# BarisYazici/deep-rl-grasping

Hardware: NVIDIA H100
Metric: SAC grad-steps/sec (batch 256, 64x64 depth) (higher is better)
Workload: dtype bf16x3 (fp32-faithful split, f32 accumulate)

## Files before the change

deep-rl-grasping_b200/csrc/engine_v2.cu:

```cuda
#include <cuda_bf16.h>

#include <algorithm>
#include <cstdio>
#include <cstdlib>
#include <cstring>

#include "sac_internal.cuh"

namespace b2g {
namespace {

struct Gather2Args {
  GatherArgs g;
  uint16_t* a1[2][3];
  uint16_t* fp[3][3];
  int KF, Ci, OH, OW;
};

__device__ __forceinline__ void split3(float y, uint16_t& p0, uint16_t& p1, uint16_t& p2) {
  const __nv_bfloat16 h0 = __float2bfloat16_rn(y);
  const float r1 = y - __bfloat162float(h0);
  const __nv_bfloat16 h1 = __float2bfloat16_rn(r1);
  const float r2 = r1 - __bfloat162float(h1);
  p0 = __bfloat16_as_ushort(h0); p1 = __bfloat16_as_ushort(h1); p2 = __bfloat16_as_ushort(__float2bfloat16_rn(r2));
}

__global__ void __launch_bounds__(512) gather2_kernel(Gather2Args a) {
  extern __shared__ uint16_t sm_planes[];
  const GatherArgs& g = a.g;
  const int b = blockIdx.x, which = blockIdx.y, tid = threadIdx.x;
  const int Ci = a.Ci, HW = g.H * g.W, npx = HW * Ci;
  const int Ec = npx + 4;
  long long slot = b;
  if (g.indices) slot = g.indices[b];
  else if (g.rng_counters) {
    slot = philox_slot(g.seed, (unsigned long long)g.rng_counters[4], b, (unsigned long long)g.rng_counters[5]);
    if (g.indices_out && which == 0 && tid == 0) g.indices_out[b] = (int)slot;
  }
  const float* __restrict__ src = (which ? g.next_obs : g.obs) + (size_t)slot * Ec;
  const double clip_obs = g.normc[1];
  const bool norm_obs = g.normc[3] != 0.0;
  const float scale = g.scale;
  const int rowe = g.W * Ci, pitch = rowe + 8, plane_e = g.H * pitch;
  for (int e4 = tid; e4 < (npx >> 2); e4 += blockDim.x) {
    const float4 v = *reinterpret_cast<const float4*>(src + 4 * e4);
    float y[4] = {v.x, v.y, v.z, v.w};
    if (norm_obs) {
      const double2 m0 = *reinterpret_cast<const double2*>(g.mean + 4 * e4), m1 = *reinterpret_cast<const double2*>(g.mean + 4 * e4 + 2);
      const double2 i0 = *reinterpret_cast<const double2*>(g.var + 4 * e4), i1 = *reinterpret_cast<const double2*>(g.var + 4 * e4 + 2);
      y[0] = (float)fmin(fmax(((double)y[0] - m0.x) * i0.x, -clip_obs), clip_obs);
      y[1] = (float)fmin(fmax(((double)y[1] - m0.y) * i0.y, -clip_obs), clip_obs);
      y[2] = (float)fmin(fmax(((double)y[2] - m1.x) * i1.x, -clip_obs), clip_obs);
      y[3] = (float)fmin(fmax(((double)y[3] - m1.y) * i1.y, -clip_obs), clip_obs);
    }
    uint16_t p[3][4];
#pragma unroll
    for (int j = 0; j < 4; ++j) split3(y[j] / scale, p[0][j], p[1][j], p[2][j]);
#pragma unroll
    for (int pl = 0; pl < 3; ++pl) {
      const uint2 w = make_uint2((uint32_t)p[pl][0] | ((uint32_t)p[pl][1] << 16), (uint32_t)p[pl][2] | ((uint32_t)p[pl][3] << 16));
      const int e = 4 * e4, row = e / rowe, col = e - row * rowe;
      *reinterpret_cast<uint2*>(sm_planes + pl * plane_e + row * pitch + col) = w;
    }
  }
  if (tid == 0) {
    float yy = src[npx];
    if (norm_obs) yy = (float)fmin(fmax(((double)yy - g.mean[npx]) * g.var[npx], -clip_obs), clip_obs);
    yy = yy / scale;
    uint16_t p0, p1, p2;
    split3(yy, p0, p1, p2);
    const size_t fo = (size_t)b * g.FS + g.feat_col, po = (size_t)b * a.KF + g.feat_col;
    if (which) { g.F_t[fo] = yy; a.fp[2][0][po] = p0; a.fp[2][1][po] = p1; a.fp[2][2][po] = p2; }
    else {
      g.F_pi[fo] = yy; g.F_v[fo] = yy;
      a.fp[0][0][po] = p0; a.fp[0][1][po] = p1; a.fp[0][2][po] = p2;
      a.fp[1][0][po] = p0; a.fp[1][1][po] = p1; a.fp[1][2][po] = p2;
    }
  }
  __syncthreads();
  const int seg = 8 * Ci;
  const int K1 = 64 * Ci, nruns = a.OH * a.OW * 8;
  const size_t img = (size_t)b * a.OH * a.OW * K1;
  for (int i = tid; i < nruns * (seg / 8); i += blockDim.x) {
    const int part = i % (seg / 8), run = i / (seg / 8);
    const int ky = run & 7, patch = run >> 3;
    const int oy = patch / a.OW, ox = patch - oy * a.OW;
    const int so = (4 * oy + ky) * pitch + 4 * ox * Ci + 8 * part;
    const size_t go = img + (size_t)patch * K1 + ky * seg + 8 * part;
#pragma unroll
    for (int pl = 0; pl < 3; ++pl) {
      const uint16_t* sp = sm_planes + pl * plane_e + so;
      const uint2 lo = *reinterpret_cast<const uint2*>(sp), hi = *reinterpret_cast<const uint2*>(sp + 4);
      *reinterpret_cast<uint4*>(a.a1[which][pl] + go) = make_uint4(lo.x, lo.y, hi.x, hi.y);
    }
  }
  if (which == 0 && g.act) {
    const int feat_dim = g.feat_col + 1;
    if (tid < g.n_act) {
      const float av = g.act[slot * g.n_act + tid];
      g.F_v[(size_t)b * g.FS + feat_dim + tid] = av;
      uint16_t p0, p1, p2;
      split3(av, p0, p1, p2);
      const size_t po = (size_t)b * a.KF + feat_dim + tid;
      a.fp[1][0][po] = p0; a.fp[1][1][po] = p1; a.fp[1][2][po] = p2;
    }
    if (tid == 32) {
      float r = g.rew[slot];
      if (g.normc[4] != 0.0) r = (float)fmin(fmax((double)r * g.normc[0], -g.normc[2]), g.normc[2]);
      g.rew_out[b] = r;
      g.done_out[b] = g.done[slot];
    }
  }
}

struct Plane2Job {
  const float* src;
  uint16_t* dst[3];
  int R, N, np;
  int transpose;
  int ld, off0;
  int tile_start;
};

__global__ void __launch_bounds__(256) planes2_kernel(const Plane2Job* __restrict__ jobs, const int* __restrict__ cta_job) {
  __shared__ float tile[64][33];
  const Plane2Job job = jobs[cta_job[blockIdx.x]];
  const int t = blockIdx.x - job.tile_start;
  const int tiles_n = (job.N + 31) / 32;
  const int r0 = (t / tiles_n) * 64, n0 = (t % tiles_n) * 32;
  const int tid = threadIdx.x;
  const bool vec_ok = (job.N & 3) == 0;
  for (int i = tid; i < 64 * 8; i += 256) {
    const int rr = i >> 3, c4 = i & 7, r = r0 + rr, n = n0 + 4 * c4;
    float4 v = make_float4(0.f, 0.f, 0.f, 0.f);
    if (r < job.R) {
      const float* sp = job.src + (size_t)r * job.N + n;
      if (vec_ok && n + 3 < job.N) v = *reinterpret_cast<const float4*>(sp);
      else { if (n < job.N) v.x = sp[0]; if (n + 1 < job.N) v.y = sp[1]; if (n + 2 < job.N) v.z = sp[2]; if (n + 3 < job.N) v.w = sp[3]; }
    }
    tile[rr][4 * c4] = v.x; tile[rr][4 * c4 + 1] = v.y; tile[rr][4 * c4 + 2] = v.z; tile[rr][4 * c4 + 3] = v.w;
    if (!job.transpose && r < job.R) {
      const float x[4] = {v.x, v.y, v.z, v.w};
      uint16_t p[3][4];
#pragma unroll
      for (int u = 0; u < 4; ++u) split3(x[u], p[0][u], p[1][u], p[2][u]);
      for (int k = 0; k < job.np; ++k) {
        uint16_t* d = job.dst[k] + (size_t)r * job.ld + job.off0 + n;
        if (n + 3 < job.N && (((size_t)r * job.ld + job.off0 + n) & 3) == 0)
          *reinterpret_cast<uint2*>(d) = make_uint2((uint32_t)p[k][0] | ((uint32_t)p[k][1] << 16), (uint32_t)p[k][2] | ((uint32_t)p[k][3] << 16));
        else
          for (int u = 0; u < 4; ++u) if (n + u < job.N) d[u] = p[k][u];
      }
    }
  }
  if (!job.transpose) return;
  __syncthreads();
  {
    const int nn = tid >> 3, g8 = tid & 7, n = n0 + nn, rb = r0 + 8 * g8;
    if (n < job.N && rb < job.R) {
      uint16_t p[3][8];
#pragma unroll
      for (int u = 0; u < 8; ++u) split3(tile[8 * g8 + u][nn], p[0][u], p[1][u], p[2][u]);
      const size_t o = (size_t)(n + job.off0) * job.ld + rb;
      for (int k = 0; k < job.np; ++k) {
        uint16_t* d = job.dst[k] + o;
        if (rb + 7 < job.R && (o & 7) == 0)
          *reinterpret_cast<uint4*>(d) = make_uint4((uint32_t)p[k][0] | ((uint32_t)p[k][1] << 16), (uint32_t)p[k][2] | ((uint32_t)p[k][3] << 16),
                                                    (uint32_t)p[k][4] | ((uint32_t)p[k][5] << 16), (uint32_t)p[k][6] | ((uint32_t)p[k][7] << 16));
        else
          for (int u = 0; u < 8; ++u) if (rb + u < job.R) d[u] = p[k][u];
      }
    }
  }
}

int add_maps(V2State& v, uint16_t* const* planes, int np, int rank, std::initializer_list<uint64_t> dims, std::initializer_list<uint64_t> strides_b,
// ... 21 lines not shown
  v.map_box_bytes.push_back((int)box_bytes);
  return (int)v.maps.size() - 1;
}

const V2State* g_mk_state = nullptr;
CgLoad mk_load(int map, int rank, int smem_off) {
  CgLoad L;
  memset(&L, 0, sizeof(L));
  L.map = map; L.rank = rank + 1; L.smem_off = smem_off;
  L.plane_box = g_mk_state->map_whole[map];
  L.box_bytes = g_mk_state->map_box_bytes[map];
  return L;
}

CgProblem kmajor(int planes, int n_tile, int chunks, int n2, int a_box_rows) {
  CgProblem P;
  memset(&P, 0, sizeof(P));
  P.tiles_m = P.tiles_n = P.splits = 1;
  P.chunks = chunks; P.n2 = n2;
  P.planes = planes;
  P.a_off = 0; P.a_pstride = 128 * 128;
  P.b_off = planes * P.a_pstride; P.b_pstride = n_tile * 128;
  P.tx_bytes = planes * (a_box_rows * 128 + n_tile * 128);
  P.mn_major = 0; P.ksteps = 4; P.a_kstep = P.b_kstep = 32;
  P.umma_n = n_tile;
  P.nprod = planes == 3 ? 6 : (planes == 2 ? 3 : 1);
  P.d0 = 1 << 20; P.d1 = 1;
  P.grp_stride = 32; P.f_grp = 32; P.bias_grp = 32;
  P.scale = 1.f;
  return P;
}

CgProblem mnmajor(int planes, int kr, int a_atoms, int b_atoms, int chunks) {
  CgProblem P;
  memset(&P, 0, sizeof(P));
  P.tiles_m = P.tiles_n = P.splits = 1;
  P.chunks = chunks; P.n2 = chunks > 0 ? chunks : 1;
  P.planes = planes;
  const int atom = kr * 128;
  P.a_off = 0; P.a_pstride = atom;
  P.b_off = 2 * planes * atom; P.b_pstride = b_atoms * atom;
  P.tx_bytes = planes * (a_atoms + b_atoms) * atom;
  P.mn_major = 1; P.ksteps = kr / 16; P.a_kstep = P.b_kstep = 2048;
  P.a_lbo = planes * atom; P.b_lbo = atom;
  P.umma_n = 64 * b_atoms;
  P.nprod = planes == 3 ? 6 : (planes == 2 ? 3 : 1);
  P.d0 = 1 << 20; P.d1 = 1;
  P.grp_stride = 32; P.f_grp = 32; P.bias_grp = 32;
  P.scale = 1.f;
  P.epi = CG_EPI_WGRAD; P.rows_tile = 128;
  return P;
}

int push_group(b2g_sac* h, std::vector<CgGroup>& list, CgGroup& g, const char* name) {
  g.name = name;
  if (cg_finalize(g, cg_smem_limit()) != 0) return b2g_fail(B2G_EINVAL, std::string("engine v2: stage ring of group ") + name + " does not fit shared memory");
  for (int i = 0; i < g.n; ++i) {
    const CgProblem& P = g.host[i];
    if (P.planes * P.umma_n > 256) return b2g_fail(B2G_EINVAL, std::string("engine v2: planes x tile width exceeds one accumulator buffer (group ") + name + ")");
    if (!cg_shape_supported(P.umma_n, P.nprod, P.mn_major != 0, P.ksteps))
      return b2g_fail(B2G_EINVAL, std::string("engine v2: no cg_kernel instance for the tile shape of a problem in group ") + name);
    g.flops += 2.0 * P.tiles_m * 128.0 * P.tiles_n * P.umma_n * P.chunks * 64.0;
  }
  list.push_back(g);
  return 0;
}

struct Wire { int cons, ci, prod, pi, dep_rows, dep_rows_tile, by_chunk; };
int fuse_groups(b2g_sac* h, const std::vector<const CgGroup*>& parts, const std::vector<Wire>& wires, const char* name, std::vector<CgGroup>& out, int& n_ctr) {
  CgGroup f;
  std::vector<int> first(parts.size());
  for (size_t gi = 0; gi < parts.size(); ++gi) {
    first[gi] = f.n;
    for (int i = 0; i < parts[gi]->n; ++i) {
      if (f.n >= CG_MAX_PROBLEMS) return b2g_fail(B2G_EINVAL, std::string("engine v2: too many problems in fused launch ") + name);
      f.host[f.n++] = parts[gi]->host[i];
    }
  }
  std::vector<int> ctr_of(f.n, -1);
  for (const Wire& w : wires) {
    const int pi = first[w.prod] + w.pi, qi = first[w.cons] + w.ci;
    CgProblem& Pp = f.host[pi];
    CgProblem& Pc = f.host[qi];
    if (Pc.dep_ctr && ctr_of[pi] < 0) {
      ctr_of[pi] = (int)(intptr_t)Pc.dep_ctr - 1;
      Pc.dep_expect += Pp.ws ? Pp.tiles_n : Pp.tiles_n * Pp.splits;
      continue;
    }
    if (Pp.splits > 1 && (Pp.splits - 1) * ((Pp.chunks + Pp.splits - 1) / Pp.splits) >= Pp.chunks)
      return b2g_fail(B2G_EINVAL, std::string("engine v2: a wired split-K producer has an empty split (fused launch ") + name + ")");
    if (ctr_of[pi] < 0) { ctr_of[pi] = n_ctr; n_ctr += Pp.tiles_m; }
    Pc.dep_rows = w.dep_rows; Pc.dep_rows_tile = w.dep_rows_tile; Pc.dep_tiles = Pp.tiles_m; Pc.dep_by_chunk = w.by_chunk;
    Pc.dep_expect = Pp.ws ? Pp.tiles_n : Pp.tiles_n * Pp.splits;
    Pc.dep_ctr = (const int*)(intptr_t)(ctr_of[pi] + 1);
  }
  for (int i = 0; i < f.n; ++i) f.host[i].done_ctr = (int*)(intptr_t)(ctr_of[i] + 1);
  return push_group(h, out, f, name);
}

void bind_counters(std::vector<CgGroup>& groups, int* base) {
  for (CgGroup& g : groups)
    for (int i = 0; i < g.n; ++i) {
      CgProblem& P = g.host[i];
      const intptr_t d = (intptr_t)P.done_ctr, c = (intptr_t)P.dep_ctr;
      P.done_ctr = d ? base + (d - 1) : nullptr;
      P.dep_ctr = c ? base + (c - 1) : nullptr;
    }
}

int check_split(const char* var, int chunks, int splits) {
  auto empty = [chunks](int s) { return (s - 1) * ((chunks + s - 1) / s) >= chunks; };
  if (!empty(splits)) return 0;
  std::string ok;
  for (int s = 1; s <= chunks; ++s)
    if (!empty(s)) ok += (ok.empty() ? "" : ", ") + std::to_string(s);
  return b2g_fail(B2G_EINVAL, std::string(var) + "=" + std::to_string(splits) + " leaves a K-split of " + std::to_string(chunks) +
                                  " chunks empty; use one of " + ok);
}

}

int v2_alloc(b2g_sac* h) {
  V2State& v = h->v2;
  const int B = h->B, Ci = h->Cimg, K1 = 64 * Ci, KF = v.KF;
  const size_t n1 = (size_t)B * 225 * 32, n2 = (size_t)B * 36 * 64, n3 = (size_t)B * 1024, na = (size_t)B * 225 * K1, nf = (size_t)B * KF;
  uint16_t *bH1, *bH2, *bH3, *bF, *bA1;
  if (int rc = dev_alloc(h->allocs, h->stream, &bH1, 9 * n1)) return rc;
  if (int rc = dev_alloc(h->allocs, h->stream, &bH2, 9 * n2)) return rc;
  if (int rc = dev_alloc(h->allocs, h->stream, &bH3, 9 * n3)) return rc;
  if (int rc = dev_alloc(h->allocs, h->stream, &bF, 9 * nf)) return rc;
  if (int rc = dev_alloc(h->allocs, h->stream, &bA1, 6 * na)) return rc;
  for (int n = 0; n < 3; ++n)
    for (int p = 0; p < 3; ++p) {
      v.H1[n][p] = bH1 + (n * 3 + p) * n1; v.H2[n][p] = bH2 + (n * 3 + p) * n2; v.H3[n][p] = bH3 + (n * 3 + p) * n3;
      v.F[n][p] = bF + (n * 3 + p) * nf;
    }
  for (int w = 0; w < 2; ++w) for (int p = 0; p < 3; ++p) v.A1[w][p] = bA1 + (w * 3 + p) * na;
  if (int rc = dev_alloc(h->allocs, h->stream, &v.z0v, (size_t)B * 3 * h->H)) return rc;
  auto palloc = [&](uint16_t** arr, int np, size_t count) -> int {
    const size_t pitch = (count + 63) / 64 * 64;
    uint16_t* base = nullptr;
    if (int rc = dev_alloc(h->allocs, h->stream, &base, pitch * np)) return rc;
    for (int p = 0; p < np; ++p) arr[p] = base + p * pitch;
    return 0;
  };
  if (int rc = palloc(v.dz0pi, 2, (size_t)B * h->H)) return rc;
  if (int rc = palloc(v.dz0v, 2, (size_t)B * 3 * h->H)) return rc;
  if (int rc = palloc(v.dZ1, 2, (size_t)B * 225 * 64)) return rc;
  for (int n = 0; n < 2; ++n) {
    if (int rc = palloc(v.dZ4[n], 2, (size_t)B * 512)) return rc;
    if (int rc = palloc(v.dZ3[n], 2, n3)) return rc;
    if (int rc = palloc(v.dZ2[n], 2, n2)) return rc;
    if (int rc = palloc(v.W2n[n], 2, 512 * 64)) return rc;
    if (int rc = palloc(v.W3n[n], 2, 576 * 64)) return rc;
    if (int rc = palloc(v.Wfn[n], 2, 1024 * 512)) return rc;
    if (int rc = palloc(v.K0n[n], 2, (size_t)KF * (n == 1 ? 3 : 1) * h->H)) return rc;
  }
  if (int rc = palloc(v.W1T[0], 3, (size_t)64 * K1)) return rc;
  if (int rc = palloc(v.W1T[1], 3, (size_t)32 * K1)) return rc;
  for (int n = 0; n < 3; ++n) {
    if (int rc = palloc(v.W2T[n], 3, 64 * 512)) return rc;
    if (int rc = palloc(v.W3T[n], 3, 64 * 576)) return rc;
    if (int rc = palloc(v.WfT[n], 3, 512 * 1024)) return rc;
    if (int rc = palloc(v.K0T[n], 3, (size_t)(n == 1 ? 3 : 1) * h->H * KF)) return rc;
  }
  return 0;
}

int v2_create(b2g_sac* h) {
  V2State& v = h->v2;
  g_mk_state = &v;
  const int B = h->B, Ci = h->Cimg, K1 = 64 * Ci, KF = v.KF, FS = h->FS, H = h->H;
  const size_t n1 = (size_t)B * 225 * 32;
  const char* nets[3] = {"model/pi", "model/values_fn", "target/values_fn"};
  std::vector<Plane2Job> jobs;
  int start = 0;
  auto add_job = [&](const float* src, int R, int N, uint16_t* const* dst, int np, int transpose, int ld, int off0) {
    Plane2Job j{};
    j.src = src; j.R = R; j.N = N; j.np = np; j.transpose = transpose; j.ld = ld; j.off0 = off0; j.tile_start = start;
    for (int k = 0; k < np; ++k) j.dst[k] = dst[k];
    start += ((R + 63) / 64) * ((N + 31) / 32);
    jobs.push_back(j);
  };
  add_job(h->p("model/pi/cnn1/w"), K1, 32, v.W1T[0], 3, 1, K1, 0);
  add_job(h->p("model/values_fn/cnn1/w"), K1, 32, v.W1T[0], 3, 1, K1, 32);
  add_job(h->p("target/values_fn/cnn1/w"), K1, 32, v.W1T[1], 3, 1, K1, 0);
  for (int n = 0; n < 3; ++n) {
    add_job(h->p(std::string(nets[n]) + "/cnn2/w"), 512, 64, v.W2T[n], 3, 1, 512, 0);
    add_job(h->p(std::string(nets[n]) + "/cnn3/w"), 576, 64, v.W3T[n], 3, 1, 576, 0);
    add_job(h->p(std::string(nets[n]) + "/cnn_fc1/w"), 1024, 512, v.WfT[n], 3, 1, 1024, 0);
  }
  add_job(h->p("model/pi/fc0/kernel"), h->feat_dim, H, v.K0T[0], 3, 1, KF, 0);
  add_job(h->p("model/values_fn/vf/fc0/kernel"), h->feat_dim, H, v.K0T[1], 3, 1, KF, 0);
  add_job(h->p("model/values_fn/qf1/fc0/kernel"), h->feat_dim + h->A, H, v.K0T[1], 3, 1, KF, H);
  add_job(h->p("model/values_fn/qf2/fc0/kernel"), h->feat_dim + h->A, H, v.K0T[1], 3, 1, KF, 2 * H);
  add_job(h->p("target/values_fn/vf/fc0/kernel"), h->feat_dim, H, v.K0T[2], 3, 1, KF, 0);
  for (int n = 0; n < 2; ++n) {
    add_job(h->p(std::string(nets[n]) + "/cnn2/w"), 512, 64, v.W2n[n], 2, 0, 64, 0);
    add_job(h->p(std::string(nets[n]) + "/cnn3/w"), 576, 64, v.W3n[n], 2, 0, 64, 0);
    add_job(h->p(std::string(nets[n]) + "/cnn_fc1/w"), 1024, 512, v.Wfn[n], 2, 0, 512, 0);
  }
  add_job(h->p("model/pi/fc0/kernel"), h->feat_dim, H, v.K0n[0], 2, 0, H, 0);
  add_job(h->p("model/values_fn/vf/fc0/kernel"), h->feat_dim, H, v.K0n[1], 2, 0, 3 * H, 0);
  add_job(h->p("model/values_fn/qf1/fc0/kernel"), h->feat_dim + h->A, H, v.K0n[1], 2, 0, 3 * H, H);
  add_job(h->p("model/values_fn/qf2/fc0/kernel"), h->feat_dim + h->A, H, v.K0n[1], 2, 0, 3 * H, 2 * H);
  v.n_plane_jobs = (int)jobs.size();
  v.plane_ctas = start;
  Plane2Job* dj = nullptr;
  if (int rc = dev_alloc(h->allocs, h->stream, &dj, jobs.size())) return rc;
  CK(cudaMemcpyAsync(dj, jobs.data(), jobs.size() * sizeof(Plane2Job), cudaMemcpyHostToDevice, h->stream));
  CK(cudaStreamSynchronize(h->stream));
  v.plane_jobs = dj;
  {
    std::vector<int> cj((size_t)start);
    for (size_t k = 0; k < jobs.size(); ++k)
      for (int t = jobs[k].tile_start; t < (k + 1 < jobs.size() ? jobs[k + 1].tile_start : start); ++t) cj[t] = (int)k;
    if (int rc = upload_table(h->allocs, h->stream, cj, &v.plane_cta_job)) return rc;
  }

  { const char* e = getenv("B2G_SPLIT_FC1"); v.split_fc1 = e ? std::max(1, atoi(e)) : 3; }
  { const char* e = getenv("B2G_SPLIT_FC1_DGRAD"); v.split_fc1_dgrad = e ? std::max(1, atoi(e)) : 1; }
  const int NP = 3;
  const long long h1_net = (long long)3 * n1;
  {
    CgGroup g;
    for (int w = 0; w < 2; ++w) {
      const int N = w == 0 ? 64 : 32;
      const int mA = add_maps(v, v.A1[w], NP, 2, {(uint64_t)K1, (uint64_t)B * 225}, {(uint64_t)K1 * 2}, {64, 128});
      const int mB = add_maps(v, v.W1T[w], NP, 2, {(uint64_t)K1, (uint64_t)N}, {(uint64_t)K1 * 2}, {64, (uint32_t)N});
      if (mA < 0 || mB < 0) return b2g_fail(B2G_ECUDA, "engine v2: cuTensorMapEncodeTiled failed (conv1)");
      CgProblem P = kmajor(NP, N, Ci, Ci, 128);
      P.nloads = 2;
      P.ld[0] = mk_load(mA, 2, 0); P.ld[0].d_tm[1] = 128; P.ld[0].d_c2[0] = 64;
      P.ld[1] = mk_load(mB, 2, P.b_off); P.ld[1].d_c2[0] = 64;
      P.tiles_m = (B * 225 + 127) / 128;
      P.epi = CG_EPI_ACT; P.rows_tile = 128; P.lim_rows = B * 225;
      P.o_tm = 128 * 32; P.o0 = 32; P.n_valid = N; P.out_planes = 3;
      P.grp_stride = (int)h1_net;
      const int net0 = w == 0 ? 0 : 2;
      for (int p = 0; p < 3; ++p) P.out_p[p] = v.H1[net0][p];
      P.bias = h->p(std::string(nets[net0]) + "/cnn1/b");
      P.bias_grp = w == 0 ? (int)(h->p("model/values_fn/cnn1/b") - h->p("model/pi/cnn1/b")) : 32;
      g.host[g.n++] = P;
    }
    if (int rc = push_group(h, v.fwd, g, "conv1_fwd")) return rc;
  }
  {
    CgGroup g;
    for (int n = 0; n < 3; ++n) {
      const int mA = add_maps(v, v.H1[n], NP, 4, {64, 14, 15, (uint64_t)B}, {64, 15 * 64, 225 * 64}, {64, 12, 12, 3}, {1, 2, 2, 1});
      const int mB = add_maps(v, v.W2T[n], NP, 2, {512, 64}, {1024}, {64, 64});
      if (mA < 0 || mB < 0) return b2g_fail(B2G_ECUDA, "engine v2: cuTensorMapEncodeTiled failed (conv2)");
      CgProblem P = kmajor(NP, 64, 8, 2, 108);
      P.nloads = 2;
      P.ld[0] = mk_load(mA, 4, 0); P.ld[0].d_tm[3] = 3; P.ld[0].d_c1[2] = 1; P.ld[0].d_c2[1] = 2;
      P.ld[1] = mk_load(mB, 2, P.b_off); P.ld[1].d_c1[0] = 128; P.ld[1].d_c2[0] = 64;
      P.tiles_m = (B + 2) / 3;
      P.epi = CG_EPI_ACT; P.rows_tile = 108; P.lim_rows = B * 36;
      P.o_tm = 108 * 64; P.o0 = 64; P.n_valid = 64; P.out_planes = 3;
      for (int p = 0; p < 3; ++p) P.out_p[p] = v.H2[n][p];
      P.bias = h->p(std::string(nets[n]) + "/cnn2/b"); P.bias_grp = 32;
      g.host[g.n++] = P;
    }
    if (int rc = push_group(h, v.fwd, g, "conv2_fwd")) return rc;
  }
  {
    CgGroup g;
    for (int n = 0; n < 3; ++n) {
      const int mA = add_maps(v, v.H2[n], NP, 4, {64, 6, 6, (uint64_t)B}, {128, 6 * 128, 36 * 128}, {64, 4, 4, 8});
      const int mB = add_maps(v, v.W3T[n], NP, 2, {576, 64}, {1152}, {64, 64});
      if (mA < 0 || mB < 0) return b2g_fail(B2G_ECUDA, "engine v2: cuTensorMapEncodeTiled failed (conv3)");
      CgProblem P = kmajor(NP, 64, 9, 3, 128);
      P.nloads = 2;
      P.ld[0] = mk_load(mA, 4, 0); P.ld[0].d_tm[3] = 8; P.ld[0].d_c1[2] = 1; P.ld[0].d_c2[1] = 1;
      P.ld[1] = mk_load(mB, 2, P.b_off); P.ld[1].d_c1[0] = 192; P.ld[1].d_c2[0] = 64;
      P.tiles_m = (B + 7) / 8;
      P.epi = CG_EPI_ACT; P.rows_tile = 128; P.lim_rows = B * 16;
      P.o_tm = 128 * 64; P.o0 = 64; P.n_valid = 64; P.out_planes = 3;
      for (int p = 0; p < 3; ++p) P.out_p[p] = v.H3[n][p];
      P.bias = h->p(std::string(nets[n]) + "/cnn3/b"); P.bias_grp = 32;
      g.host[g.n++] = P;
    }
    if (int rc = push_group(h, v.fwd, g, "conv3_fwd")) return rc;
  }
  {
    CgGroup g;
    for (int n = 0; n < 3; ++n) {
      const int mA = add_maps(v, v.H3[n], NP, 2, {1024, (uint64_t)B}, {2048}, {64, 128});
      const int mB = add_maps(v, v.WfT[n], NP, 2, {1024, 512}, {2048}, {64, 64});
      if (mA < 0 || mB < 0) return b2g_fail(B2G_ECUDA, "engine v2: cuTensorMapEncodeTiled failed (cnn_fc1)");
      CgProblem P = kmajor(NP, 64, 16, 16, 128);
      P.nloads = 2;
      P.ld[0] = mk_load(mA, 2, 0); P.ld[0].d_tm[1] = 128; P.ld[0].d_c2[0] = 64;
      P.ld[1] = mk_load(mB, 2, P.b_off); P.ld[1].d_tn[1] = 64; P.ld[1].d_c2[0] = 64;
      P.tiles_m = (B + 127) / 128; P.tiles_n = 8;
      P.epi = CG_EPI_ACT; P.rows_tile = 128; P.lim_rows = B;
      P.o_tm = (long long)128 * KF; P.o0 = KF; P.n_valid = 512; P.out_planes = 3;
      for (int p = 0; p < 3; ++p) P.out_p[p] = v.F[n][p];
      P.bias = h->p(std::string(nets[n]) + "/cnn_fc1/b"); P.bias_grp = 32;
      P.out_f = h->F[n]; P.f_tm = (long long)128 * FS; P.f0 = FS; P.f_grp = 32;
      if (v.split_fc1 > 1) {
        P.splits = v.split_fc1;
        if (int rc = check_split("B2G_SPLIT_FC1", P.chunks, P.splits)) return rc;
        if (int rc = dev_alloc(h->allocs, h->stream, &P.ws, (size_t)P.tiles_m * P.tiles_n * 128 * 64)) return rc;
        if (int rc = dev_alloc(h->allocs, h->stream, &P.ws_cnt, (size_t)P.tiles_m * P.tiles_n * CG_EPI_WARPS)) return rc;
      }
      g.host[g.n++] = P;
    }
    if (int rc = push_group(h, v.fwd, g, "fc1_fwd")) return rc;
  }
  {
    CgGroup g;
    float* z0out[3] = {h->z0[0], v.z0v, h->z0[4]};
    for (int n = 0; n < 3; ++n) {
      const int Nn = n == 1 ? 3 * H : H;
      const int mA = add_maps(v, v.F[n], NP, 2, {(uint64_t)KF, (uint64_t)B}, {(uint64_t)KF * 2}, {64, 128});
      const int mB = add_maps(v, v.K0T[n], NP, 2, {(uint64_t)KF, (uint64_t)Nn}, {(uint64_t)KF * 2}, {64, 64});
      if (mA < 0 || mB < 0) return b2g_fail(B2G_ECUDA, "engine v2: cuTensorMapEncodeTiled failed (fc0)");
      CgProblem P = kmajor(NP, 64, KF / 64, KF / 64, 128);
      P.nloads = 2;
      P.ld[0] = mk_load(mA, 2, 0); P.ld[0].d_tm[1] = 128; P.ld[0].d_c2[0] = 64;
      P.ld[1] = mk_load(mB, 2, P.b_off); P.ld[1].d_tn[1] = 64; P.ld[1].d_c2[0] = 64;
      P.tiles_m = (B + 127) / 128; P.tiles_n = Nn / 64;
      P.epi = CG_EPI_RAW; P.rows_tile = 128; P.lim_rows = B;
      P.o_tm = (long long)128 * Nn; P.o0 = Nn; P.n_valid = Nn;
      P.splits = P.chunks; P.atomic = 1;
// ... 51 lines not shown
        }
        g.host[g.n++] = P;
      }
      {
        const int mA = add_maps(v, v.H3[n], NB, 2, {1024, (uint64_t)B}, {2048}, {64, 64});
        const int mB = add_maps(v, v.dZ4[n], NB, 2, {512, (uint64_t)B}, {1024}, {64, 64}, {}, false);
        if (mA < 0 || mB < 0) return b2g_fail(B2G_ECUDA, "engine v2: cuTensorMapEncodeTiled failed (fc1 wgrad)");
        CgProblem P = mnmajor(NB, 64, 2, 2, (B + 63) / 64);
        P.nloads = 4;
        for (int a = 0; a < 2; ++a) {
          P.ld[a] = mk_load(mA, 2, a * P.a_lbo); P.ld[a].c0[0] = 64 * a; P.ld[a].d_tm[0] = 128; P.ld[a].d_c2[1] = 64;
          P.ld[2 + a] = mk_load(mB, 2, P.b_off + a * 8192); P.ld[2 + a].c0[0] = 64 * a; P.ld[2 + a].d_tn[0] = 128; P.ld[2 + a].d_c2[1] = 64;
        }
        P.tiles_m = 8; P.tiles_n = 4;
        P.lim_rows = 1024; P.o_tm = 128 * 512; P.o0 = 512; P.n_valid = 512;
        P.out_f = h->g(std::string(nets[n]) + "/cnn_fc1/w"); P.atomic = 0;
        g.host[g.n++] = P;
      }
    }
    if (int rc = push_group(h, v.bwd_groups, g, "fc1_bwd")) return rc;
  }
  {
    CgGroup g;
    std::vector<int> tab(5 * CG_MAX_LOADS * 2, 0);
    for (int tm = 0; tm < 5; ++tm)
      for (int a = 0; a < 2; ++a) {
        const int pos = 2 * tm + a;
        tab[(tm * CG_MAX_LOADS + a) * 2] = pos % 3; tab[(tm * CG_MAX_LOADS + a) * 2 + 1] = pos / 3;
      }
    const int* dtab = nullptr;
    if (int rc = upload_table(h->allocs, h->stream, tab, &dtab)) return rc;
    for (int n = 0; n < 2; ++n) {
      {
        const int mA = add_maps(v, v.dZ3[n], NB, 4, {64, 4, 4, (uint64_t)B}, {128, 512, 2048}, {64, 6, 6, 3});
        const int mB = add_maps(v, v.W3n[n], NB, 2, {64, 576}, {128}, {64, 64});
        if (mA < 0 || mB < 0) return b2g_fail(B2G_ECUDA, "engine v2: cuTensorMapEncodeTiled failed (conv3 dgrad)");
        CgProblem P = kmajor(NB, 64, 9, 3, 108);
        P.nloads = 2;
        P.ld[0] = mk_load(mA, 4, 0); P.ld[0].d_tm[3] = 3; P.ld[0].d_c1[2] = -1; P.ld[0].d_c2[1] = -1;
        P.ld[1] = mk_load(mB, 2, P.b_off); P.ld[1].d_c1[1] = 192; P.ld[1].d_c2[1] = 64;
        P.tiles_m = (B + 2) / 3;
        P.epi = CG_EPI_DGRAD; P.rows_tile = 108; P.lim_rows = B * 36;
        P.o_tm = 108 * 64; P.o0 = 64; P.n_valid = 64; P.out_planes = 2;
        for (int p = 0; p < 2; ++p) P.out_p[p] = v.dZ2[n][p];
        P.mask = v.H2[n][0]; P.m_tm = 108 * 64; P.m0 = 64;
        P.colsum = h->g(std::string(nets[n]) + "/cnn2/b"); P.colsum_mask = 63;
        g.host[g.n++] = P;
      }
      {
        const int mA = add_maps(v, v.H2[n], NB, 4, {64, 6, 6, (uint64_t)B}, {128, 768, 4608}, {64, 4, 4, 4});
        const int mB = add_maps(v, v.dZ3[n], NB, 2, {64, (uint64_t)B * 16}, {128}, {64, 64});
        if (mA < 0 || mB < 0) return b2g_fail(B2G_ECUDA, "engine v2: cuTensorMapEncodeTiled failed (conv3 wgrad)");
        CgProblem P = mnmajor(NB, 64, 2, 1, (B + 3) / 4);
        P.nloads = 3;
        for (int a = 0; a < 2; ++a) { P.ld[a] = mk_load(mA, 4, a * P.a_lbo); P.ld[a].d_c2[3] = 4; }
        P.ld[2] = mk_load(mB, 2, P.b_off); P.ld[2].d_c2[1] = 64;
        P.tm_tab = dtab;
        P.tiles_m = 5; P.tiles_n = 1;
        P.splits = std::max(1, std::min(P.chunks, std::max(14, (P.chunks + 15) / 16)));
        P.lim_rows = 576; P.o_tm = 128 * 64; P.o0 = 64; P.n_valid = 64;
        P.out_f = h->g(std::string(nets[n]) + "/cnn3/w"); P.atomic = 1;
        g.host[g.n++] = P;
      }
    }
    if (int rc = push_group(h, v.bwd_groups, g, "conv3_bwd")) return rc;
  }
  {
    CgGroup g;
    for (int n = 0; n < 2; ++n) {
      const int mA = add_maps(v, v.dZ2[n], NB, 4, {64, 6, 6, (uint64_t)B}, {128, 768, 4608}, {64, 8, 8, 2});
      const int mB = add_maps(v, v.W2n[n], NB, 2, {64, 512}, {128}, {64, 64}, {}, false);
      if (mA < 0 || mB < 0) return b2g_fail(B2G_ECUDA, "engine v2: cuTensorMapEncodeTiled failed (conv2 dgrad)");
      CgProblem P = kmajor(NB, 128, 4, 2, 128);
      P.tx_bytes = NB * (128 * 128 + 2 * 64 * 128);
      P.nloads = 3;
      P.ld[0] = mk_load(mA, 4, 0); P.ld[0].d_tm[3] = 2; P.ld[0].d_c1[2] = -1; P.ld[0].d_c2[1] = -1;
      for (int py = 0; py < 2; ++py) {
        P.ld[1 + py] = mk_load(mB, 2, P.b_off + py * 64 * 128);
        P.ld[1 + py].c0[1] = py * 128; P.ld[1 + py].d_c1[1] = 256; P.ld[1 + py].d_c2[1] = 64;
      }
      P.tiles_m = (B + 1) / 2;
      P.epi = CG_EPI_DGRAD; P.rows_tile = 128; P.lim_rows = B * 64;
      P.d0 = 8; P.d1 = 8;
      P.o_tm = 2 * 225 * 64; P.o0 = 2 * 64; P.o1 = 2 * 15 * 64; P.o2 = 225 * 64; P.o_base = n * 32;
      P.m_tm = 2 * 225 * 32; P.m0 = 2 * 32; P.m1 = 2 * 15 * 32; P.m2 = 225 * 32; P.m_base = 0;
      P.grp_tab = 1;
      for (int py = 0; py < 2; ++py)
        for (int px = 0; px < 2; ++px) {
          const int gg = py * 2 + px;
          P.grp_off[gg] = (py * 15 + px) * 64; P.grp_moff[gg] = (py * 15 + px) * 32;
          P.grp_lim0[gg] = (15 - px + 1) / 2; P.grp_lim1[gg] = (15 - py + 1) / 2;
        }
      P.n_valid = 128; P.out_planes = 2;
      for (int p = 0; p < 2; ++p) P.out_p[p] = v.dZ1[p];
      P.mask = v.H1[n][0];
      P.colsum = h->g(std::string(nets[n]) + "/cnn1/b"); P.colsum_mask = 31;
      g.host[g.n++] = P;
    }
    if (int rc = push_group(h, v.bwd_groups, g, "conv2_dgrad")) return rc;
  }
  {
    CgGroup g;
    for (int n = 0; n < 2; ++n) {
      const int mA = add_maps(v, v.H1[n], NB, 4, {64, 14, 15, (uint64_t)B}, {64, 15 * 64, 225 * 64}, {64, 12, 12, 4}, {1, 2, 2, 1});
      const int mB = add_maps(v, v.dZ2[n], NB, 2, {64, (uint64_t)B * 36}, {128}, {64, 144});
      if (mA < 0 || mB < 0) return b2g_fail(B2G_ECUDA, "engine v2: cuTensorMapEncodeTiled failed (conv2 wgrad)");
      CgProblem P = mnmajor(NB, 144, 2, 1, (B + 3) / 4);
      P.nloads = 3;
      for (int a = 0; a < 2; ++a) { P.ld[a] = mk_load(mA, 4, a * P.a_lbo); P.ld[a].c0[1] = 2 * a; P.ld[a].d_tm[2] = 1; P.ld[a].d_c2[3] = 4; }
      P.ld[2] = mk_load(mB, 2, P.b_off); P.ld[2].d_c2[1] = 144;
      P.tiles_m = 4; P.tiles_n = 1;
      P.splits = std::max(1, std::min(P.chunks, std::max(8, (P.chunks + 7) / 8)));
      P.lim_rows = 512; P.o_tm = 128 * 64; P.o0 = 64; P.n_valid = 64;
      P.out_f = h->g(std::string(nets[n]) + "/cnn2/w"); P.atomic = 1;
      g.host[g.n++] = P;
    }
    {
      const int mA = add_maps(v, v.A1[0], NB, 2, {(uint64_t)K1, (uint64_t)B * 225}, {(uint64_t)K1 * 2}, {64, 64});
      const int mB = add_maps(v, v.dZ1, NB, 2, {64, (uint64_t)B * 225}, {128}, {64, 64});
      if (mA < 0 || mB < 0) return b2g_fail(B2G_ECUDA, "engine v2: cuTensorMapEncodeTiled failed (conv1 wgrad)");
      CgProblem P = mnmajor(NB, 64, 2, 1, (B * 225 + 63) / 64);
      P.nloads = 3;
      for (int a = 0; a < 2; ++a) { P.ld[a] = mk_load(mA, 2, a * P.a_lbo); P.ld[a].c0[0] = 64 * a; P.ld[a].d_tm[0] = 128; P.ld[a].d_c2[1] = 64; }
      P.ld[2] = mk_load(mB, 2, P.b_off); P.ld[2].d_c2[1] = 64;
      P.tiles_m = (K1 + 127) / 128; P.tiles_n = 1;
      P.splits = std::max(1, std::min(P.chunks, std::max(84 / P.tiles_m, (P.chunks + 15) / 16)));
      P.lim_rows = K1; P.o_tm = 128 * 32; P.o0 = 32; P.n_valid = 64;
      P.out_f = h->g("model/pi/cnn1/w"); P.f_grp = (long long)(h->g("model/values_fn/cnn1/w") - h->g("model/pi/cnn1/w")); P.atomic = 1;
      g.host[g.n++] = P;
    }
    if (int rc = push_group(h, v.bwd_groups, g, "conv_wgrad")) return rc;
  }
  int n_ctr = 0;
  {
    std::vector<const CgGroup*> parts;
    for (auto& g : v.fwd) parts.push_back(&g);
    std::vector<Wire> w;
    for (int n = 0; n < 3; ++n) {
      w.push_back({1, n, 0, n < 2 ? 0 : 1, 3 * 225, 128, 0});
      w.push_back({2, n, 1, n, 8 * 36, 108, 0});
      w.push_back({3, n, 2, n, 128 * 16, 128, 0});
      w.push_back({4, n, 3, n, 128, 128, 0});
    }
    if (int rc = fuse_groups(h, parts, w, "fwd_fused", v.fwd_fused, n_ctr)) return rc;
  }
  {
    std::vector<const CgGroup*> parts;
    for (auto& g : v.bwd_groups) parts.push_back(&g);
    std::vector<Wire> w;
    for (int n = 0; n < 2; ++n) {
      w.push_back({1, 2 * n, 0, n, 128, 128, 0});
      w.push_back({1, 2 * n + 1, 0, n, 64, 128, 1});
      w.push_back({2, 2 * n, 1, 2 * n, 3, 128, 0});
      w.push_back({2, 2 * n + 1, 1, 2 * n, 4, 128, 1});
      w.push_back({3, n, 2, 2 * n, 72, 108, 0});
      w.push_back({4, n, 2, 2 * n, 144, 108, 1});
    }
    w.push_back({4, 2, 3, 0, 64, 450, 1});
    w.push_back({4, 2, 3, 1, 64, 450, 1});
    if (int rc = fuse_groups(h, parts, w, "bwd_fused", v.bwd_fused, n_ctr)) return rc;
    std::vector<const CgGroup*> pa(parts.begin(), parts.begin() + 2), pb(parts.begin() + 2, parts.end());
    std::vector<Wire> wa, wb;
    for (int n = 0; n < 2; ++n) {
      wa.push_back({1, 2 * n, 0, n, 128, 128, 0});
      wa.push_back({1, 2 * n + 1, 0, n, 64, 128, 1});
      wb.push_back({1, n, 0, 2 * n, 72, 108, 0});
      wb.push_back({2, n, 0, 2 * n, 144, 108, 1});
    }
    wb.push_back({2, 2, 1, 0, 64, 450, 1});
    wb.push_back({2, 2, 1, 1, 64, 450, 1});
    if (int rc = fuse_groups(h, pa, wa, "bwd_fused_fc", v.bwd_fused, n_ctr)) return rc;
    if (int rc = fuse_groups(h, pb, wb, "bwd_fused_conv", v.bwd_fused, n_ctr)) return rc;
  }
  if (int rc = dev_alloc(h->allocs, h->stream, &v.dep_ctr, (size_t)n_ctr)) return rc;
  v.n_dep_ctr = n_ctr;
  bind_counters(v.fwd_fused, v.dep_ctr);
  bind_counters(v.bwd_fused, v.dep_ctr);
  if (int rc = dev_alloc(h->allocs, h->stream, &v.d_maps, v.maps.size())) return rc;
  CK(cudaMemcpyAsync(v.d_maps, v.maps.data(), v.maps.size() * sizeof(CUtensorMap), cudaMemcpyHostToDevice, h->stream));
  CK(cudaStreamSynchronize(h->stream));
  return 0;
}

int v2_planes(b2g_sac* h, cudaStream_t s) {
  V2State& v = h->v2;
  planes2_kernel<<<v.plane_ctas, 256, 0, s>>>((const Plane2Job*)v.plane_jobs, v.plane_cta_job);
  return 0;
}

int v2_gather(b2g_sac* h, const GatherArgs& ga, cudaStream_t s) {
  V2State& v = h->v2;
  Gather2Args a{};
  a.g = ga;
  for (int w = 0; w < 2; ++w)
    for (int p = 0; p < 3; ++p) a.a1[w][p] = v.A1[w][p];
  for (int n = 0; n < 3; ++n) for (int p = 0; p < 3; ++p) a.fp[n][p] = v.F[n][p];
  a.KF = v.KF; a.Ci = h->Cimg; a.OH = h->H1; a.OW = h->W1;
  const size_t smem = (size_t)3 * h->Hi * (h->Wi * h->Cimg + 8) * sizeof(uint16_t);
  static size_t attr = 0;
  if (smem > attr) {
    CK(cudaFuncSetAttribute(gather2_kernel, cudaFuncAttributeMaxDynamicSharedMemorySize, (int)smem));
    attr = smem;
  }
  gather2_kernel<<<dim3(ga.B, ga.next_obs ? 2 : 1), 512, smem, s>>>(a);
  return 0;
}

extern long long* g_cg_trace;
static long long* s_trace_buf = nullptr;

int v2_launch(b2g_sac* h, const CgGroup& g, cudaStream_t s) {
  const char* tn = getenv("B2G_CG_TRACE");
  cudaStreamCaptureStatus cs0 = cudaStreamCaptureStatusNone;
  if (tn) cudaStreamIsCapturing(s, &cs0);
  if (tn && cs0 == cudaStreamCaptureStatusNone && std::string(tn) == g.name) {
    if (!s_trace_buf) cudaMalloc(&s_trace_buf, 640 * sizeof(long long));
    cudaMemsetAsync(s_trace_buf, 0, 640 * sizeof(long long), s);
    g_cg_trace = s_trace_buf;
    const char* tc = getenv("B2G_CG_TRACE_CTA");
    cudaError_t e = cg_launch(g, h->v2.d_maps, h->num_sms - h->v2.sm_reserve, s, false, h->v2.dbg | ((tc ? atoi(tc) : 0) << 8));
    g_cg_trace = nullptr;
    if (e != cudaSuccess) return b2g_fail(B2G_ECUDA, cudaGetErrorString(e));
    static int shots = 0;
    if (shots++ == 3) {
      long long t[640];
      cudaStreamSynchronize(s);
      cudaMemcpy(t, s_trace_buf, sizeof(t), cudaMemcpyDeviceToHost);
      const long long t0 = t[0];
      fprintf(stderr, "cg trace %s (cycles; per chunk: prod wait_start wait_done issued | mma wait_start full_seen committed)\n", g.name);
      for (int i = 0; i < 64 && t[i * 8 + 2]; ++i)
        fprintf(stderr, "  chunk %2d (p %lld tm %lld): %7lld %7lld %7lld | %7lld %7lld %7lld\n", i, t[i * 8 + 6] / 100000, t[i * 8 + 6] % 100000 / 10, t[i * 8] - t0,
                t[i * 8 + 1] - t0, t[i * 8 + 2] - t0, t[i * 8 + 3] - t0, t[i * 8 + 4] - t0, t[i * 8 + 5] - t0);
      for (int i = 0; i < 16 && t[512 + i * 4 + 2]; ++i)
        fprintf(stderr, "  tile %d (p %lld tm %lld) epilogue: wait_start %7lld acc_full %7lld done %7lld | first group: ld issued %7lld ld done %7lld math done %7lld\n", i,
                t[512 + i * 4 + 3] / 100000, t[512 + i * 4 + 3] % 100000 / 10, t[512 + i * 4] - t0, t[512 + i * 4 + 1] - t0, t[512 + i * 4 + 2] - t0,
                t[576 + i * 4] - t0, t[576 + i * 4 + 1] - t0, t[576 + i * 4 + 2] - t0);
    }
    return 0;
  }
  CK(cg_launch(g, h->v2.d_maps, h->num_sms - h->v2.sm_reserve, s, pdl_enabled(), h->v2.dbg));
  return 0;
}

}
```

deep-rl-grasping_b200/csrc/sac_internal.cuh:

```cuda
#pragma once
#include <cuda_runtime.h>

#include <map>
#include <string>
#include <tuple>
#include <vector>

#include "../../include/b200grasp.h"
#include "cg.cuh"
#include "common.cuh"
#include "host.cuh"

namespace b2g {
struct Tensor {
  std::string name;
  int ndim;
  int64_t shape[4];
  int64_t numel;
  int64_t off;
  int group;
};


struct V2State {
  bool on = false;
  int KF = 576;
  uint16_t* A1[2][3]{};
  uint16_t* H1[3][3]{};
  uint16_t* H2[3][3]{};
  uint16_t* H3[3][3]{};
  uint16_t* F[3][3]{};
  uint16_t* dz0pi[2]{};
  uint16_t* dz0v[2]{};
  uint16_t* dZ4[2][2]{};
  uint16_t* dZ3[2][2]{};
  uint16_t* dZ2[2][2]{};
  uint16_t* dZ1[2]{};
  uint16_t* W1T[2][3]{};
  uint16_t* W2T[3][3]{};
  uint16_t* W3T[3][3]{};
  uint16_t* WfT[3][3]{};
  uint16_t* K0T[3][3]{};
  uint16_t* W2n[2][2]{};
  uint16_t* W3n[2][2]{};
  uint16_t* Wfn[2][2]{};
  uint16_t* K0n[2][2]{};
  float* z0v = nullptr;
  void* plane_jobs = nullptr; int n_plane_jobs = 0, plane_ctas = 0;
  const int* plane_cta_job = nullptr;
  int sm_reserve = 0;
  std::vector<CUtensorMap> maps;
  std::vector<char> map_whole;
  std::vector<int> map_box_bytes;
  CUtensorMap* d_maps = nullptr;
  std::vector<CgGroup> fwd, bwd_groups;
  std::vector<CgGroup> fwd_fused, bwd_fused;
  int split_fc1 = 3;
  int split_fc1_dgrad = 1;
  int* dep_ctr = nullptr; int n_dep_ctr = 0;
  std::vector<int*> tabs;
  int dbg = 0;
};

}

struct b2g_sac;
namespace b2g {
int v2_alloc(b2g_sac* h);
int v2_create(b2g_sac* h);
int v2_planes(b2g_sac* h, cudaStream_t s);
int v2_gather(b2g_sac* h, const GatherArgs& ga, cudaStream_t s);
int v2_launch(b2g_sac* h, const CgGroup& g, cudaStream_t s);
}

using namespace b2g;

struct b2g_sac {
  b2g_sac_cfg cfg{};
  bool cnn = false;
  int num_sms = 132;
  int B = 0, A = 0, H = 0, E = 0, Cimg = 0, feat_dim = 0, FS = 0;
  int Hi = 0, Wi = 0, H1 = 0, W1 = 0, H2 = 0, W2 = 0, H3 = 0, W3 = 0;
  std::vector<Tensor> tensors;
  std::map<std::string, int> tindex;
  int64_t n_pi = 0, n_values = 0, n_ent = 0, n_target = 0, n_train = 0, n_all = 0;
  float *P = nullptr, *Mo = nullptr, *Vo = nullptr, *G = nullptr;
  float* metrics = nullptr;
  cudaStream_t stream = nullptr;
  std::vector<void*> allocs;
  int Ec = 0;
  float *r_obs = nullptr, *r_next = nullptr, *r_act = nullptr, *r_rew = nullptr, *r_done = nullptr;
  int64_t r_size = 0, r_pos = 0;
  float* obs_stage = nullptr;
  int stage_rows = 0;
  double *d_mean = nullptr, *d_istd = nullptr, *d_normc = nullptr;
  double ret_istd = 1.0, clip_obs = 10.0, clip_rew = 10.0;
  int norm_obs = 0, norm_rew = 0;
  float *x_obs = nullptr, *x_next = nullptr;
  float *h1[3]{}, *h2[3]{}, *h3[3]{}, *F[3]{};
  float *dZ4[2]{}, *dZ3p[2]{}, *dZ2p[2]{}, *dZ1[2]{};
  float *z0[5]{}, *a0[4]{}, *dz1[4]{}, *dz0_pi = nullptr, *dz0_v3 = nullptr;
  bool use_planes = false;
  uint16_t *xp[2][2]{}, *h1p[3][2]{}, *h2p[3][2]{}, *h3p[3][2]{};
  uint16_t *dZ4p[2][2]{}, *dZ3pp[2][2]{}, *dZ2pp[2][2]{}, *dZ1p[2][2]{};
  ColsumJob* d_colsum = nullptr;
  int n_colsum = 0, colsum_ctas = 0;
  uint16_t* wp[3][4][4]{};
  PlaneJob* d_jobs = nullptr;
  int n_jobs = 0, job_tiles = 0;
  bool planes_dirty = true;
// ... 59 lines not shown
```

Baseline: 2130.

## Replace materialized conv1 im2col with column-band buffer read via 4D TMA maps

The gather kernel no longer writes the full im2col matrix (225 patches × 64·Ci per image) for conv1. It writes one 8-column band per output column, and the conv1 forward and wgrad GEMMs read overlapping windows through 4D tensor maps. This cuts the gather's global write traffic and buffer size roughly by the 8x8 patch overlap factor. In exchange, the conv1 forward is split into two half problems with per-image tiles, and the dependency wiring, output and dgrad offset tables are remapped, which adds risk of tile-shape inefficiency or indexing errors.

```diff
diff --git a/deep-rl-grasping_b200/csrc/engine_v2.cu b/deep-rl-grasping_b200/csrc/engine_v2.cu
--- a/deep-rl-grasping_b200/csrc/engine_v2.cu
+++ b/deep-rl-grasping_b200/csrc/engine_v2.cu
@@ -12,7 +12,7 @@
 
 struct Gather2Args {
   GatherArgs g;
-  uint16_t* a1[2][3];
+  uint16_t* xb[2][3];
   uint16_t* fp[3][3];
   int KF, Ci, OH, OW;
 };
@@ -78,20 +78,18 @@
     }
   }
   __syncthreads();
-  const int seg = 8 * Ci;
-  const int K1 = 64 * Ci, nruns = a.OH * a.OW * 8;
-  const size_t img = (size_t)b * a.OH * a.OW * K1;
-  for (int i = tid; i < nruns * (seg / 8); i += blockDim.x) {
+  const int seg = 8 * Ci, band_e = g.H * seg;
+  const size_t img = (size_t)b * 16 * band_e;
+  for (int i = tid; i < a.OW * band_e / 8; i += blockDim.x) {
     const int part = i % (seg / 8), run = i / (seg / 8);
-    const int ky = run & 7, patch = run >> 3;
-    const int oy = patch / a.OW, ox = patch - oy * a.OW;
-    const int so = (4 * oy + ky) * pitch + 4 * ox * Ci + 8 * part;
-    const size_t go = img + (size_t)patch * K1 + ky * seg + 8 * part;
+    const int ox = run / g.H, y = run - ox * g.H;
+    const int so = y * pitch + 4 * ox * Ci + 8 * part;
+    const size_t go = img + (size_t)ox * band_e + y * seg + 8 * part;
 #pragma unroll
     for (int pl = 0; pl < 3; ++pl) {
       const uint16_t* sp = sm_planes + pl * plane_e + so;
       const uint2 lo = *reinterpret_cast<const uint2*>(sp), hi = *reinterpret_cast<const uint2*>(sp + 4);
-      *reinterpret_cast<uint4*>(a.a1[which][pl] + go) = make_uint4(lo.x, lo.y, hi.x, hi.y);
+      *reinterpret_cast<uint4*>(a.xb[which][pl] + go) = make_uint4(lo.x, lo.y, hi.x, hi.y);
     }
   }
   if (which == 0 && g.act) {
@@ -279,8 +277,10 @@
     const int pi = first[w.prod] + w.pi, qi = first[w.cons] + w.ci;
     CgProblem& Pp = f.host[pi];
     CgProblem& Pc = f.host[qi];
-    if (Pc.dep_ctr && ctr_of[pi] < 0) {
-      ctr_of[pi] = (int)(intptr_t)Pc.dep_ctr - 1;
+    if (Pc.dep_ctr) {
+      const int c = (int)(intptr_t)Pc.dep_ctr - 1;
+      if (ctr_of[pi] < 0) ctr_of[pi] = c;
+      else if (ctr_of[pi] != c) return b2g_fail(B2G_EINVAL, std::string("engine v2: producers of one consumer signal different counters (fused launch ") + name + ")");
       Pc.dep_expect += Pp.ws ? Pp.tiles_n : Pp.tiles_n * Pp.splits;
       continue;
     }
@@ -320,19 +320,19 @@
 int v2_alloc(b2g_sac* h) {
   V2State& v = h->v2;
   const int B = h->B, Ci = h->Cimg, K1 = 64 * Ci, KF = v.KF;
-  const size_t n1 = (size_t)B * 225 * 32, n2 = (size_t)B * 36 * 64, n3 = (size_t)B * 1024, na = (size_t)B * 225 * K1, nf = (size_t)B * KF;
-  uint16_t *bH1, *bH2, *bH3, *bF, *bA1;
+  const size_t n1 = (size_t)B * 225 * 32, n2 = (size_t)B * 36 * 64, n3 = (size_t)B * 1024, nb = (size_t)B * 16 * 8 * K1, nf = (size_t)B * KF;
+  uint16_t *bH1, *bH2, *bH3, *bF, *bXB;
   if (int rc = dev_alloc(h->allocs, h->stream, &bH1, 9 * n1)) return rc;
   if (int rc = dev_alloc(h->allocs, h->stream, &bH2, 9 * n2)) return rc;
   if (int rc = dev_alloc(h->allocs, h->stream, &bH3, 9 * n3)) return rc;
   if (int rc = dev_alloc(h->allocs, h->stream, &bF, 9 * nf)) return rc;
-  if (int rc = dev_alloc(h->allocs, h->stream, &bA1, 6 * na)) return rc;
+  if (int rc = dev_alloc(h->allocs, h->stream, &bXB, 6 * nb)) return rc;
   for (int n = 0; n < 3; ++n)
     for (int p = 0; p < 3; ++p) {
       v.H1[n][p] = bH1 + (n * 3 + p) * n1; v.H2[n][p] = bH2 + (n * 3 + p) * n2; v.H3[n][p] = bH3 + (n * 3 + p) * n3;
       v.F[n][p] = bF + (n * 3 + p) * nf;
     }
-  for (int w = 0; w < 2; ++w) for (int p = 0; p < 3; ++p) v.A1[w][p] = bA1 + (w * 3 + p) * na;
+  for (int w = 0; w < 2; ++w) for (int p = 0; p < 3; ++p) v.XB[w][p] = bXB + (w * 3 + p) * nb;
   if (int rc = dev_alloc(h->allocs, h->stream, &v.z0v, (size_t)B * 3 * h->H)) return rc;
   auto palloc = [&](uint16_t** arr, int np, size_t count) -> int {
     const size_t pitch = (count + 63) / 64 * 64;
@@ -419,26 +419,32 @@
   { const char* e = getenv("B2G_SPLIT_FC1_DGRAD"); v.split_fc1_dgrad = e ? std::max(1, atoi(e)) : 1; }
   const int NP = 3;
   const long long h1_net = (long long)3 * n1;
+  if (h1_net > INT32_MAX) return b2g_fail(B2G_EINVAL, "engine v2: batch too large for the conv1 output offsets");
   {
     CgGroup g;
     for (int w = 0; w < 2; ++w) {
       const int N = w == 0 ? 64 : 32;
-      const int mA = add_maps(v, v.A1[w], NP, 2, {(uint64_t)K1, (uint64_t)B * 225}, {(uint64_t)K1 * 2}, {64, 128});
+      const int mA = add_maps(v, v.XB[w], NP, 4, {(uint64_t)K1, 15, 8, (uint64_t)B * 2}, {(uint64_t)K1, (uint64_t)K1 * 16, (uint64_t)K1 * 128}, {64, 16, 8, 1});
       const int mB = add_maps(v, v.W1T[w], NP, 2, {(uint64_t)K1, (uint64_t)N}, {(uint64_t)K1 * 2}, {64, (uint32_t)N});
       if (mA < 0 || mB < 0) return b2g_fail(B2G_ECUDA, "engine v2: cuTensorMapEncodeTiled failed (conv1)");
-      CgProblem P = kmajor(NP, N, Ci, Ci, 128);
-      P.nloads = 2;
-      P.ld[0] = mk_load(mA, 2, 0); P.ld[0].d_tm[1] = 128; P.ld[0].d_c2[0] = 64;
-      P.ld[1] = mk_load(mB, 2, P.b_off); P.ld[1].d_c2[0] = 64;
-      P.tiles_m = (B * 225 + 127) / 128;
-      P.epi = CG_EPI_ACT; P.rows_tile = 128; P.lim_rows = B * 225;
-      P.o_tm = 128 * 32; P.o0 = 32; P.n_valid = N; P.out_planes = 3;
-      P.grp_stride = (int)h1_net;
       const int net0 = w == 0 ? 0 : 2;
-      for (int p = 0; p < 3; ++p) P.out_p[p] = v.H1[net0][p];
-      P.bias = h->p(std::string(nets[net0]) + "/cnn1/b");
-      P.bias_grp = w == 0 ? (int)(h->p("model/values_fn/cnn1/b") - h->p("model/pi/cnn1/b")) : 32;
-      g.host[g.n++] = P;
+      for (int half = 0; half < 2; ++half) {
+        CgProblem P = kmajor(NP, N, Ci, Ci, 128);
+        P.nloads = 2;
+        P.ld[0] = mk_load(mA, 4, 0); P.ld[0].c0[3] = half; P.ld[0].d_tm[3] = 2; P.ld[0].d_c2[0] = 64;
+        P.ld[1] = mk_load(mB, 2, P.b_off); P.ld[1].d_c2[0] = 64;
+        P.tiles_m = B;
+        P.epi = CG_EPI_ACT; P.rows_tile = 128; P.lim_rows = B * 128;
+        P.d0 = 16; P.d1 = 8;
+        P.o_tm = 225 * 32; P.o0 = 15 * 32; P.o1 = 32; P.o_base = half * 8 * 32;
+        P.grp_tab = 1;
+        for (int gg = 0; gg < N / 32; ++gg) { P.grp_off[gg] = (int)(gg * h1_net); P.grp_lim0[gg] = 15; P.grp_lim1[gg] = 8 - half; }
+        P.n_valid = N; P.out_planes = 3;
+        for (int p = 0; p < 3; ++p) P.out_p[p] = v.H1[net0][p];
+        P.bias = h->p(std::string(nets[net0]) + "/cnn1/b");
+        P.bias_grp = w == 0 ? (int)(h->p("model/values_fn/cnn1/b") - h->p("model/pi/cnn1/b")) : 32;
+        g.host[g.n++] = P;
+      }
     }
     if (int rc = push_group(h, v.fwd, g, "conv1_fwd")) return rc;
   }
@@ -656,13 +662,13 @@
       P.tiles_m = (B + 1) / 2;
       P.epi = CG_EPI_DGRAD; P.rows_tile = 128; P.lim_rows = B * 64;
       P.d0 = 8; P.d1 = 8;
-      P.o_tm = 2 * 225 * 64; P.o0 = 2 * 64; P.o1 = 2 * 15 * 64; P.o2 = 225 * 64; P.o_base = n * 32;
+      P.o_tm = 2 * 225 * 64; P.o0 = 2 * 15 * 64; P.o1 = 2 * 64; P.o2 = 225 * 64; P.o_base = n * 32;
       P.m_tm = 2 * 225 * 32; P.m0 = 2 * 32; P.m1 = 2 * 15 * 32; P.m2 = 225 * 32; P.m_base = 0;
       P.grp_tab = 1;
       for (int py = 0; py < 2; ++py)
         for (int px = 0; px < 2; ++px) {
           const int gg = py * 2 + px;
-          P.grp_off[gg] = (py * 15 + px) * 64; P.grp_moff[gg] = (py * 15 + px) * 32;
+          P.grp_off[gg] = (px * 15 + py) * 64; P.grp_moff[gg] = (py * 15 + px) * 32;
           P.grp_lim0[gg] = (15 - px + 1) / 2; P.grp_lim1[gg] = (15 - py + 1) / 2;
         }
       P.n_valid = 128; P.out_planes = 2;
@@ -690,13 +696,16 @@
       g.host[g.n++] = P;
     }
     {
-      const int mA = add_maps(v, v.A1[0], NB, 2, {(uint64_t)K1, (uint64_t)B * 225}, {(uint64_t)K1 * 2}, {64, 64});
-      const int mB = add_maps(v, v.dZ1, NB, 2, {64, (uint64_t)B * 225}, {128}, {64, 64});
+      const int mA = add_maps(v, v.XB[0], NB, 4, {(uint64_t)K1, 15, 16, (uint64_t)B}, {(uint64_t)K1, (uint64_t)K1 * 16, (uint64_t)K1 * 256}, {64, 16, 4, 1});
+      const int mB = add_maps(v, v.dZ1, NB, 4, {64, 15, 15, (uint64_t)B}, {128, 15 * 128, 225 * 128}, {64, 16, 4, 1});
       if (mA < 0 || mB < 0) return b2g_fail(B2G_ECUDA, "engine v2: cuTensorMapEncodeTiled failed (conv1 wgrad)");
-      CgProblem P = mnmajor(NB, 64, 2, 1, (B * 225 + 63) / 64);
+      CgProblem P = mnmajor(NB, 64, 2, 1, 4 * B);
+      P.n2 = 4;
       P.nloads = 3;
-      for (int a = 0; a < 2; ++a) { P.ld[a] = mk_load(mA, 2, a * P.a_lbo); P.ld[a].c0[0] = 64 * a; P.ld[a].d_tm[0] = 128; P.ld[a].d_c2[1] = 64; }
-      P.ld[2] = mk_load(mB, 2, P.b_off); P.ld[2].d_c2[1] = 64;
+      for (int a = 0; a < 2; ++a) {
+        P.ld[a] = mk_load(mA, 4, a * P.a_lbo); P.ld[a].c0[0] = 64 * a; P.ld[a].d_tm[0] = 128; P.ld[a].d_c1[3] = 1; P.ld[a].d_c2[2] = 4;
+      }
+      P.ld[2] = mk_load(mB, 4, P.b_off); P.ld[2].d_c1[3] = 1; P.ld[2].d_c2[2] = 4;
       P.tiles_m = (K1 + 127) / 128; P.tiles_n = 1;
       P.splits = std::max(1, std::min(P.chunks, std::max(84 / P.tiles_m, (P.chunks + 15) / 16)));
       P.lim_rows = K1; P.o_tm = 128 * 32; P.o0 = 32; P.n_valid = 64;
@@ -711,7 +720,8 @@
     for (auto& g : v.fwd) parts.push_back(&g);
     std::vector<Wire> w;
     for (int n = 0; n < 3; ++n) {
-      w.push_back({1, n, 0, n < 2 ? 0 : 1, 3 * 225, 128, 0});
+      for (int half = 0; half < 2; ++half)
+        w.push_back({1, n, 0, (n < 2 ? 0 : 2) + half, 3, 1, 0});
       w.push_back({2, n, 1, n, 8 * 36, 108, 0});
       w.push_back({3, n, 2, n, 128 * 16, 128, 0});
       w.push_back({4, n, 3, n, 128, 128, 0});
@@ -730,8 +740,8 @@
       w.push_back({3, n, 2, 2 * n, 72, 108, 0});
       w.push_back({4, n, 2, 2 * n, 144, 108, 1});
     }
-    w.push_back({4, 2, 3, 0, 64, 450, 1});
-    w.push_back({4, 2, 3, 1, 64, 450, 1});
+    w.push_back({4, 2, 3, 0, 1, 8, 1});
+    w.push_back({4, 2, 3, 1, 1, 8, 1});
     if (int rc = fuse_groups(h, parts, w, "bwd_fused", v.bwd_fused, n_ctr)) return rc;
     std::vector<const CgGroup*> pa(parts.begin(), parts.begin() + 2), pb(parts.begin() + 2, parts.end());
     std::vector<Wire> wa, wb;
@@ -741,8 +751,8 @@
       wb.push_back({1, n, 0, 2 * n, 72, 108, 0});
       wb.push_back({2, n, 0, 2 * n, 144, 108, 1});
     }
-    wb.push_back({2, 2, 1, 0, 64, 450, 1});
-    wb.push_back({2, 2, 1, 1, 64, 450, 1});
+    wb.push_back({2, 2, 1, 0, 1, 8, 1});
+    wb.push_back({2, 2, 1, 1, 1, 8, 1});
     if (int rc = fuse_groups(h, pa, wa, "bwd_fused_fc", v.bwd_fused, n_ctr)) return rc;
     if (int rc = fuse_groups(h, pb, wb, "bwd_fused_conv", v.bwd_fused, n_ctr)) return rc;
   }
@@ -767,7 +777,7 @@
   Gather2Args a{};
   a.g = ga;
   for (int w = 0; w < 2; ++w)
-    for (int p = 0; p < 3; ++p) a.a1[w][p] = v.A1[w][p];
+    for (int p = 0; p < 3; ++p) a.xb[w][p] = v.XB[w][p];
   for (int n = 0; n < 3; ++n) for (int p = 0; p < 3; ++p) a.fp[n][p] = v.F[n][p];
   a.KF = v.KF; a.Ci = h->Cimg; a.OH = h->H1; a.OW = h->W1;
   const size_t smem = (size_t)3 * h->Hi * (h->Wi * h->Cimg + 8) * sizeof(uint16_t);
diff --git a/deep-rl-grasping_b200/csrc/sac_internal.cuh b/deep-rl-grasping_b200/csrc/sac_internal.cuh
--- a/deep-rl-grasping_b200/csrc/sac_internal.cuh
+++ b/deep-rl-grasping_b200/csrc/sac_internal.cuh
@@ -25,7 +25,7 @@
 struct V2State {
   bool on = false;
   int KF = 576;
-  uint16_t* A1[2][3]{};
+  uint16_t* XB[2][3]{};
   uint16_t* H1[3][3]{};
   uint16_t* H2[3][3]{};
   uint16_t* H3[3][3]{};
```

Result: faster. 2153, median of 6 (+1.1%).
